# wei-zeng98/piano-a2s

Measured on AMD Instinct MI355X. Metric: training clips/sec (12 s, 5-bar), higher is better.
Workload: dtype f32

## Files before the change

### piano_a2s_amd/csrc/a2s_api.hip

```cpp
#define A2S_SWITCHES_IMPL
#include "a2s_internal.h"

thread_local char a2s_err_msg[512] = {0};
long long a2s_launch_counter = 0;

#define ST ((hipStream_t)stream)

extern "C" {

const char* a2s_last_error(void) { return a2s_err_msg; }
int a2s_version(void) { return 1; }
long long a2s_launch_count(void) { return __atomic_load_n(&a2s_launch_counter, __ATOMIC_RELAXED); }

int a2s_gemm_f32(void* stream, int M, int N, int K, float alpha, const float* A, long sAm, long sAk, const float* B, long sBk,
                 long sBn, float beta, float* C, long ldc, const float* bias, int act, int batch, long bsA, long bsB, long bsC,
                 int splitk, float* workspace, size_t workspace_bytes) {
    return a2s_gemm_impl(ST, M, N, K, alpha, A, sAm, sAk, B, sBk, sBn, beta, C, ldc, bias, act, batch, bsA, bsB, bsC, splitk,
                         workspace, workspace_bytes);
}
int a2s_gemm_f32_affine(void* stream, int M, int N, int K, float alpha, const float* A, long sAm, long sAk, const float* B, long sBk,
                        long sBn, float beta, float* C, long ldc, const float* bias, int act, int batch, long bsA, long bsB, long bsC,
                        int splitk, float* workspace, size_t workspace_bytes, const float* a_scale, const float* a_shift, int a_period,
                        const float* b_scale, const float* b_shift, int b_period) {
    return a2s_gemm_affine_impl(ST, M, N, K, alpha, A, sAm, sAk, B, sBk, sBn, beta, C, ldc, bias, act, batch, bsA, bsB, bsC, splitk,
// ... 32 lines not shown
}
size_t a2s_linear_wgrad_ws_bytes(int M, int K) { return a2s_linear_wgrad_ws_bytes_impl(M, K); }
int a2s_linear_wgrad_eligible(int M, int N, int K, int period) { return a2s_linear_wgrad_ok(M, N, K, 256, 4, 4, period, nullptr, nullptr, nullptr) ? 1 : 0; }
int a2s_tallk_wgrad(void* stream, int M, int Np, int K, const float* P, long ldp, const float* A, long lda, float* G, long ldg, int transposed, float* bias,
                    const float* p_absmax, const float* a_absmax, float* workspace, size_t workspace_bytes) {
    return a2s_tallk_wgrad_impl(ST, M, Np, K, P, ldp, A, lda, G, ldg, transposed, bias, p_absmax, a_absmax, workspace, workspace_bytes);
}
size_t a2s_tallk_wgrad_ws_bytes(int M, int Np, int K) { return a2s_tallk_wgrad_ws_bytes_impl(M, Np, K); }
int a2s_tallk_wgrad_eligible(int M, int Np, int K, long ldp, long lda, long ldg, int transposed) {
    return a2s_tallk_wgrad_ok(M, Np, K, ldp, lda, ldg, transposed, nullptr, nullptr, nullptr, nullptr) ? 1 : 0;
}
int a2s_linear_fwd_eligible(int M, int N, int K, int period) { return a2s_linear_fwd_ok(M, N, K, 4, 4, period, nullptr, nullptr, nullptr) ? 1 : 0; }
int a2s_linear_dgrad_blocks(int M) { return a2s_linear_dgrad_blocks_impl(M); }
int a2s_linear_dgrad_eligible(int M, int N, int K, int period) {
    return a2s_linear_dgrad_ok(M, N, K, 4, 1, K, 4, period, nullptr, nullptr, nullptr, nullptr) ? 1 : 0;
}
int a2s_gemm_f32_bnstats(void* stream, int M, int N, int K, const float* A, long sAm, long sAk, const float* B, long sBk, long sBn, float* C, long ldc,
                         const float* y, const float* mean, const float* invstd, const float* scale, const float* shift, int period, float* partial) {
    return a2s_gemm_affine_impl(ST, M, N, K, 1.f, A, sAm, sAk, B, sBk, sBn, 0.f, C, ldc, nullptr, 0, 1, 0, 0, 0, 1, nullptr, 0,
                                nullptr, nullptr, 0, nullptr, nullptr, 0, y, mean, invstd, scale, shift, partial, period, 0, nullptr, nullptr);
}
int a2s_gemm_bnstats_blocks(int M, int period) { return a2s_cdiv(M, 128) * a2s_gemm_bnstats_slots(period); }
size_t a2s_gemm_workspace_bytes(int M, int N, int batch, int splitk) { return a2s_gemm_workspace_bytes_impl(M, N, batch, splitk); }
int a2s_gemm_pick_splitk(int M, int N, int K, int batch) { return a2s_gemm_pick_splitk_impl(M, N, K, batch); }
void a2s_gemm_debug_tile(int cfg) { a2s_gemm_debug_tile_impl(cfg); }
size_t a2s_note_step_workspace_floats(int H, int E) { return a2s_note_step_workspace_floats_impl(H, E); }
int a2s_debug_set(const char* key, int value) {
    if (!key) return A2S_ERR_ARG;
    const int id = a2s_switch_find(key);
    if (id >= 0) { a2s_switch_store(id, value); return A2S_OK; }
    if (!strcmp(key, "attn_deferred_fast")) { a2s_attn_deferred_fast = value ? 1 : 0; return A2S_OK; }
    if (!strcmp(key, "tallk_wgrad")) { a2s_tallk_wgrad_on = value ? 1 : 0; return A2S_OK; }
    if (!strcmp(key, "tallk_wgrad_max_splits")) { a2s_tallk_wgrad_max_splits = value > 0 ? value : 0; return A2S_OK; }
    if (!strcmp(key, "gemm_tile")) { a2s_gemm_debug_tile_impl(value); return A2S_OK; }
    snprintf(a2s_err_msg, sizeof(a2s_err_msg), "a2s_debug_set: unknown key %s", key);
    return A2S_ERR_ARG;
}
int a2s_env_check(void) {
    if (const char* e = a2s_switch_env_error()) A2S_FAIL(A2S_ERR_ARG, "%s: expected a decimal number >= 0", e);
    return A2S_OK;
}

int a2s_persist_abort_latch(void* device_word) { a2s_persist_latch_set(device_word); return A2S_OK; }

int a2s_debug_get(const char* key) {
    if (!key) return -1;
    const int id = a2s_switch_find(key);
    if (id == A2S_SW_attn_pair_fused_rows) return a2s_attn_pair_fused_rows();
    if (id >= 0) return a2s_sw((a2s_switch)id);
    if (!strcmp(key, "attn_pair_launches")) return (int)a2s_attn_pair_launches();
    if (!strcmp(key, "attn_pair_bwd_launches")) return (int)a2s_attn_pair_bwd_launches();
    if (!strcmp(key, "attn_deferred_fast")) return a2s_attn_deferred_fast;
    if (!strcmp(key, "tallk_wgrad")) return a2s_tallk_wgrad_on;
    if (!strcmp(key, "tallk_wgrad_max_splits")) return a2s_tallk_wgrad_max_splits;
    if (!strcmp(key, "tallk_wgrad_launches")) return (int)a2s_tallk_wgrad_launches();
    if (!strcmp(key, "attn_dk_ahead_launches")) return (int)a2s_attn_dk_ahead_launches();
    if (!strcmp(key, "attn_denc_launches")) return (int)a2s_attn_denc_launches();
    if (!strcmp(key, "dec_mid_launches")) return a2s_dec_mid_launches();
    if (!strcmp(key, "dec_cmb_launches")) return a2s_dec_cmb_launches();
    if (!strcmp(key, "dec_persist_launches")) return a2s_dec_persist_launches();
    if (!strcmp(key, "gru_persist_fwd_launches")) return (int)a2s_gru_persist_fwd_launches();
    if (!strcmp(key, "gru_persist_bwd_launches")) return (int)a2s_gru_persist_bwd_launches();
    if (!strcmp(key, "gru_step_fwd_launches")) return (int)a2s_gru_step_fwd_launches();
    if (!strcmp(key, "gru_step_bwd_launches")) return (int)a2s_gru_step_bwd_launches();
    if (!strcmp(key, "edit_distance_launches")) return (int)a2s_edit_distance_launches();
    if (!strcmp(key, "conv_rows16_c20_launches")) return (int)a2s_conv_rows16_c20_launches();
    if (!strcmp(key, "device_cus")) return a2s_device_geometry().cus;
    if (!strcmp(key, "device_xccs")) return a2s_device_geometry().xccs;
    return -1;
}

int a2s_conv3x3(void* stream, const float* x, const float* w, float* y, const float* in_scale, const float* in_shift,
                float* stat_partial, int B, int T, int F, int Cin, int Cout, int flip, float* workspace) {
    return a2s_conv3x3_impl(ST, x, w, y, in_scale, in_shift, stat_partial, B, T, F, Cin, Cout, flip, workspace, nullptr, nullptr, nullptr, nullptr, nullptr, nullptr,
                            nullptr, nullptr);
}
int a2s_conv3x3_ranged(void* stream, const float* x, const float* w, float* y, const float* in_scale, const float* in_shift, const float* in_absmax,
                       float* stat_partial, float* out_absmax, int B, int T, int F, int Cin, int Cout, float* workspace) {
    return a2s_conv3x3_impl(ST, x, w, y, in_scale, in_shift, stat_partial, B, T, F, Cin, Cout, 0, workspace, nullptr, nullptr, nullptr, nullptr, nullptr, nullptr,
                            in_absmax, out_absmax);
}
int a2s_conv3x3_dgrad_bnstats(void* stream, const float* dy, const float* w, float* g, const float* yl, const float* yl_mean, const float* yl_invstd,
                              const float* yl_scale, const float* yl_shift, float* stat_partial, int B, int T, int F, int Cin, int Cout,
                              float* workspace) {
    if (!yl) { snprintf(a2s_err_msg, sizeof(a2s_err_msg), "conv3x3_dgrad_bnstats: yl is required"); return A2S_ERR_ARG; }
    return a2s_conv3x3_impl(ST, dy, w, g, nullptr, nullptr, stat_partial, B, T, F, Cin, Cout, 1, workspace, yl, yl_mean, yl_invstd, yl_scale, yl_shift, nullptr, nullptr, nullptr);
}
int a2s_conv3x3_dgrad_bnstats_scaled(void* stream, const float* dy, const float* w, float* g, const float* yl, const float* yl_mean, const float* yl_invstd,
                                     const float* yl_scale, const float* yl_shift, float* stat_partial, int B, int T, int F, int Cin, int Cout,
                                     float* workspace, const float* dy_absmax) {
    if (!yl) { snprintf(a2s_err_msg, sizeof(a2s_err_msg), "conv3x3_dgrad_bnstats_scaled: yl is required"); return A2S_ERR_ARG; }
    return a2s_conv3x3_impl(ST, dy, w, g, nullptr, nullptr, stat_partial, B, T, F, Cin, Cout, 1, workspace, yl, yl_mean, yl_invstd, yl_scale, yl_shift, dy_absmax, nullptr, nullptr);
}
int a2s_conv3x3_dgrad_bnstats_ranged(void* stream, const float* dy, const float* w, float* g, const float* yl, const float* yl_mean, const float* yl_invstd,
                                     const float* yl_scale, const float* yl_shift, float* stat_partial, int B, int T, int F, int Cin, int Cout,
                                     float* workspace, const float* dy_absmax, float* g_absmax_out) {
    if (!yl) { snprintf(a2s_err_msg, sizeof(a2s_err_msg), "conv3x3_dgrad_bnstats_ranged: yl is required"); return A2S_ERR_ARG; }
    return a2s_conv3x3_impl(ST, dy, w, g, nullptr, nullptr, stat_partial, B, T, F, Cin, Cout, 1, workspace, yl, yl_mean, yl_invstd, yl_scale, yl_shift, dy_absmax, nullptr, g_absmax_out);
}
// ... 395 lines not shown
```

### piano_a2s_amd/csrc/a2s_conv_rows.hip

```cpp
#include "a2s_internal.h"
#include <type_traits>

#define RW_P 120
#define RW_SROW 288
#define RW_SLOTS 5
#ifndef RW_EB
#define RW_EB 4
#endif
#define RW_HDR 160

typedef short s16x4 __attribute__((ext_vector_type(4)));
typedef short s16x8 __attribute__((ext_vector_type(8)));
#define RW_LDS(p) ((__attribute__((address_space(3))) s16x4*)(p))

template <int CIN>
struct RwGeom {
    static constexpr int NB = CIN / 4;
    static constexpr int KS = (3 * NB + 7) / 8;
    static constexpr int TS = CIN * RW_SROW;
    static constexpr int SLOT = 2 * TS + (CIN % 8 ? 128 : 0);
    static constexpr int ITEMS = CIN * 32;
    static constexpr int XIT = (ITEMS + 255) / 256;
};

// ... 518 lines not shown
        if (co >= 0)
            for (int e = tid; e < CIN * 9; e += 256) m = fmaxf(m, fabsf(weight(co, e / 9, e % 9)));
        m = block_max(m, red);
        if (tid == 0) {
            kw[c] = pow2_scale_exp(m, 13);
            if (co >= 0 && df == 0) hdr[80 + co] = ldexpf(1.f, -kw[c]);
        }
        __syncthreads();
    }
    for (int idx = tid; idx < G::KS * 512; idx += 256) {
        const int s = idx / 512, lane = (idx >> 3) & 63, e8 = idx & 7;
        const int li = lane & 15, g = lane >> 4, r = e8 >> 2, e = e8 & 3;
        const int kb = 8 * s + 4 * r + g;
        int co, df;
        column(li, co, df);
        float v = 0.f;
        if (co >= 0 && kb < 3 * G::NB) v = ldexpf(weight(co, 4 * (kb % G::NB) + e, (kb / G::NB) * 3 + df), kw[li]);
        unsigned t0, t1;
        split2_pair_f16(v, 0.f, t0, t1);
        unsigned short* dst = reinterpret_cast<unsigned short*>(wimg + ((size_t)(tile * G::KS + s) * 2) * 1024 + lane * 16 + e8 * 2);
        dst[0] = (unsigned short)t0;
        dst[512] = (unsigned short)t1;
    }
}

__device__ __forceinline__ float rw_ror8(float x) {
    return __int_as_float(__builtin_amdgcn_update_dpp(0, __float_as_int(x), 0x128, 0xf, 0xf, true));
}
__device__ __forceinline__ float rw_rol4(float x) {
    return __int_as_float(__builtin_amdgcn_update_dpp(0, __float_as_int(x), 0x12c, 0xf, 0xf, true));
}

#define R16_SLOTS 4
template <int CIN, int COUT, bool AFFINE, bool BNRED, bool PIPE = false>
__global__ __launch_bounds__(512, 2) void conv3x3_rows16(RowsArgs a) {
    using G = RwGeom<CIN>;
    using N = R16Geom<COUT>;
    constexpr int NTHR = 512, KS = G::KS;
    constexpr int WNM = N::WNM, NNT = N::NNT;
    constexpr bool B1L = PIPE || (CIN == 20 && COUT == 20 && BNRED);
    constexpr int XIT = (G::ITEMS + NTHR - 1) / NTHR;
    __shared__ __attribute__((aligned(16))) unsigned char ring[R16_SLOTS * G::SLOT];
    __shared__ __attribute__((aligned(16))) unsigned char b1img[B1L ? N::NTILES * G::KS * 1024 : 16];
    __shared__ float xch[2][N::NBND][2][16];
    __shared__ float red[8][16][3];
    __shared__ float tab[(AFFINE ? 2 * CIN : 0) + (BNRED ? 4 * COUT : 0) + 4];
    __shared__ __attribute__((aligned(16))) unsigned char dump[(G::ITEMS % NTHR) ? NTHR * 16 : 16];

    const int tid = threadIdx.x, lane = tid & 63;
    const int wave = __builtin_amdgcn_readfirstlane(tid >> 6);
    const int q = lane & 15, g = lane >> 4;
    const bool wide = wave < 4;
    const int wg = wave / N::WSPLIT, rng = wave % N::WSPLIT;
    const int m0 = wide ? WNM * rng : 2 * (wave - 4);
    const int nm = wide ? WNM : 2;
    const int tile0 = wide ? 3 * wg : 3 * N::NWG;
    const bool neg = wave & 1;
    const float sg = neg ? -1.f : 1.f;
    const int bnd_l = wide ? (rng > 0 ? wg * (N::WSPLIT - 1) + rng - 1 : -1) : (wave > 4 ? N::NWB + wave - 5 : -1);
    const int bnd_r = wide ? (rng < N::WSPLIT - 1 ? wg * (N::WSPLIT - 1) + rng : -1) : (wave < 7 ? N::NWB + wave - 4 : -1);

    int bid = blockIdx.x;
    {
        const int per = (int)gridDim.x / 8;
        if (bid < per * 8) bid = (bid % 8) * per + bid / 8;
    }
    const int ft = bid % a.tilesF; bid /= a.tilesF;
    const int strip = bid % a.nstrips, b = bid / a.nstrips;
    const int f_base = ft * RW_P;
    const int t_lo = strip * a.strip_len, t_hi = min(a.T, t_lo + a.strip_len);

    const unsigned sgn = neg ? 0x80008000u : 0u;
    constexpr int BWT = B1L ? 1 : 2;
    s16x8 bw[3][KS][BWT];
#pragma unroll
    for (int d = 0; d < 3; ++d)
#pragma unroll
        for (int s = 0; s < KS; ++s)
#pragma unroll
            for (int tm = 0; tm < BWT; ++tm) {
// ... 7 lines not shown
    }
    auto bterm1 = [&](int d, int s) -> s16x8 {
        if (B1L) {
            uint4 v = *reinterpret_cast<const uint4*>(b1img + ((tile0 + ((wide || d < NNT) ? d : 0)) * KS + s) * 1024 + lane * 16);
            v.x ^= sgn; v.y ^= sgn; v.z ^= sgn; v.w ^= sgn;
            return __builtin_bit_cast(s16x8, v);
        }
        return bw[d][s][BWT - 1];
    };
    const int co = wide ? wg * 16 + q : 16 * N::NWG + (q & (N::R - 1));
    const bool useful = wide || q < N::R;
    const float xscale = a.hdr[120];
    const float unsc = useful ? a.hdr[80 + co] / xscale * sg : 0.f;
    if (AFFINE && tid < 2 * CIN) tab[tid] = a.hdr[tid < CIN ? tid : 40 + tid - CIN];
    if (BNRED && tid < 4 * COUT) {
        const float* src = tid < COUT ? a.yl_mean : tid < 2 * COUT ? a.yl_invstd : tid < 3 * COUT ? a.yl_scale : a.yl_shift;
        tab[tid] = src[tid % COUT];
    }
    __syncthreads();
    float bm = 0.f, bi = 0.f, bsc = 0.f, bsh = 0.f;
    if (BNRED && useful) { bm = tab[co]; bi = tab[COUT + co]; bsc = tab[2 * COUT + co]; bsh = tab[3 * COUT + co]; }
    f32x2 st_s = {0.f, 0.f}, st_s2 = {0.f, 0.f};
    float st_m = 0.f;

    unsigned aaddr[KS][2];
#pragma unroll
    for (int s = 0; s < KS; ++s)
#pragma unroll
        for (int r = 0; r < 2; ++r) {
            int dt, cb;
            rw_block<CIN>(8 * s + 4 * r + g, dt, cb);
            aaddr[s][r] = (unsigned)(dt * G::SLOT + (4 * cb + q / 4) * RW_SROW + (q % 4) * 8 + m0 * 32);
        }
    const float* __restrict__ xclip = a.x + (long)b * a.T * CIN * a.F;
    const __amdgpu_buffer_rsrc_t xrsrc = __builtin_amdgcn_make_buffer_rsrc(const_cast<float*>(xclip), 0, (unsigned)((long)a.T * CIN * a.F * 4), 0x00020000);
    typedef unsigned u32x4 __attribute__((ext_vector_type(4)));
    const int fcol = f_base - 4 + 4 * (tid & 31);
    const bool colok = fcol >= 0 && fcol < a.F;
    auto issue = [&](int row, f32x4 (&xr)[XIT]) {
        const int rbase = row * CIN * a.F + f_base - 4;
        int tl = tid;
        asm volatile("" : "+v"(tl));
#pragma unroll
        for (int it = 0; it < XIT; ++it) {
            const int e = tl + NTHR * it;
            const int goff = (e >> 5) * a.F + 4 * (e & 31) + rbase;
            xr[it] = __builtin_bit_cast(f32x4, __builtin_amdgcn_raw_buffer_load_b128(xrsrc, (colok && e < G::ITEMS) ? goff * 4 : -4, 0, 0));
        }
    };
    auto commit_item = [&](int it, bool ok, unsigned char* base, const f32x4& x) {
        int tl = tid;
        asm volatile("" : "+v"(tl));
        const int e = tl + NTHR * it;
        const bool has = (it + 1) * NTHR <= G::ITEMS || e < G::ITEMS;
        const int ch = has ? e >> 5 : 0;
        unsigned char* const p0 = has ? base + ch * RW_SROW + (e & 31) * 8 : dump + tl * 16;
        unsigned char* const p1 = has ? p0 + G::TS : p0 + 8;
        f32x4 v = x;
        if (AFFINE) {
            const float sc = tab[ch], sh = tab[CIN + ch];
#pragma unroll
            for (int k = 0; k < 4; ++k) v[k] = ok ? fmaxf(fmaf(v[k], sc, sh), 0.f) : 0.f;
        } else {
#pragma unroll
            for (int k = 0; k < 4; ++k) v[k] = ok ? v[k] * xscale : 0.f;
        }
        uint2 t0, t1;
        split2_pair_f16(v[0], v[1], t0.x, t1.x);
        split2_pair_f16(v[2], v[3], t0.y, t1.y);
        *reinterpret_cast<uint2*>(p0) = t0;
        *reinterpret_cast<uint2*>(p1) = t1;
    };

    f32x4 acc[WNM][3];
    auto dterm1 = [](auto WIDEc, const f32x4 t0, const f32x4 t1, int r) -> float {
        if constexpr (decltype(WIDEc)::value) return t1[r];
        else if constexpr (N::R == 8) return rw_ror8(t0[r]);
        else return rw_rol4(t0[r]);
    };
    auto dterm2 = [](auto WIDEc, const f32x4 t0, const f32x4 t1, const f32x4 t2, int r) -> float {
        if constexpr (decltype(WIDEc)::value) return t2[r];
        else if constexpr (N::R == 8) return t1[r];
        else return rw_ror8(t0[r]);
    };
    auto multiply = [&](auto NMc, auto NTc, int crow, int cslot, const f32x4 (&xr)[XIT]) {
        constexpr int NM = decltype(NMc)::value, NT = decltype(NTc)::value;
        const bool cok = crow >= 0 && crow < a.T && colok;
        unsigned char* const cbase = ring + cslot * G::SLOT;
#pragma unroll
        for (int i = 0; i < NM; ++i)
#pragma unroll
            for (int d = 0; d < NT; ++d) acc[i][d] = (f32x4){0.f, 0.f, 0.f, 0.f};
#pragma unroll
        for (int s = 0; s < KS; ++s) {
            s16x8 b1[NT];
#pragma unroll
            for (int d = 0; d < NT; ++d) b1[d] = bterm1(d, s);
#pragma unroll
            for (int ig = 0; ig < NM / 2; ++ig) {
                s16x8 av[2][2];
#pragma unroll
                for (int tm = 0; tm < 2; ++tm)
#pragma unroll
                    for (int ii = 0; ii < 2; ++ii) {
                        const int off = tm * G::TS + (ig * 2 + ii) * 32;
                        const s16x4 lo = __builtin_amdgcn_ds_read_tr16_b64_v4i16(RW_LDS(ring + aaddr[s][0] + off));
                        const s16x4 hi = __builtin_amdgcn_ds_read_tr16_b64_v4i16(RW_LDS(ring + aaddr[s][1] + off));
                        av[tm][ii] = __builtin_shufflevector(lo, hi, 0, 1, 2, 3, 4, 5, 6, 7);
                    }
#define R16_PRODUCT(TA, BV)                                                                                                  \
    _Pragma("unroll") for (int d = 0; d < NT; ++d)                                                                           \
        _Pragma("unroll") for (int ii = 0; ii < 2; ++ii)                                                                     \
            acc[ig * 2 + ii][d] = __builtin_amdgcn_mfma_f32_16x16x32_f16(__builtin_bit_cast(f16x8, av[TA][ii]), __builtin_bit_cast(f16x8, BV), acc[ig * 2 + ii][d], 0, 0, 0);
                R16_PRODUCT(1, bw[d][s][0])
                R16_PRODUCT(0, b1[d])
                R16_PRODUCT(0, bw[d][s][0])
#undef R16_PRODUCT
            }
#pragma unroll
            for (int it = 0; it < XIT; ++it)
                if (it * KS / XIT == s) commit_item(it, cok, cbase, xr[it]);
        }
    };
    auto advance = [&]() {
#pragma unroll
        for (int s = 0; s < KS; ++s)
#pragma unroll
            for (int r = 0; r < 2; ++r) {
                const unsigned n = aaddr[s][r] + G::SLOT;
                aaddr[s][r] = min(n, n - R16_SLOTS * G::SLOT);
            }
    };

    const int up_addr = (((g + 3) & 3) * 16 + q) * 4;
    const int dn_addr = (((g + 1) & 3) * 16 + q) * 4;
    unsigned okbits = 0;
#pragma unroll
    for (int i = 0; i < WNM; ++i) {
        const int p = 16 * (m0 + i) + 4 * g;
        if (useful && i < nm && p >= 4 && p < 4 + RW_P && f_base - 4 + p < a.F) okbits |= 1u << i;
    }
    const __amdgpu_buffer_rsrc_t yrsrc = __builtin_amdgcn_make_buffer_rsrc(a.y + (long)b * a.T * COUT * a.F, 0, (unsigned)((long)a.T * COUT * a.F * 4), 0x00020000);
    const __amdgpu_buffer_rsrc_t ylrsrc = __builtin_amdgcn_make_buffer_rsrc(const_cast<float*>(BNRED ? a.yl + (long)b * a.T * COUT * a.F : a.x), 0,
                                                                            BNRED ? (unsigned)((long)a.T * COUT * a.F * 4) : 0u, 0x00020000);
    const int yvo = (co * a.F + f_base - 4 + 16 * m0 + 4 * g) * 4;
    f32x4 ylv[BNRED ? WNM : 1];
    auto yl_fetch = [&](int t) {
        if (!BNRED) return;
        const int yrow_off = t * COUT * a.F * 4;
#pragma unroll
        for (int i = 0; i < WNM; ++i)
            if (i < nm) ylv[BNRED ? i : 0] = __builtin_bit_cast(f32x4, __builtin_amdgcn_raw_buffer_load_b128(ylrsrc, yvo + 64 * i, yrow_off, 0));
    };
    auto epilogue = [&](auto WIDEc, int t, int par) {
// ... 19 lines not shown
            const float us = ok ? unsc : 0.f;
            f32x4 d1;
#pragma unroll
            for (int r = 0; r < 4; ++r) d1[r] = dterm1(WIDEc, acc[i][0], acc[i][1], r);
            f32x4 o;
            o[0] = ((X[i] + d1[0]) + dterm2(WIDEc, acc[i][0], acc[i][1], acc[i][2], 1)) * us;
            o[1] = ((acc[i][0][0] + d1[1]) + dterm2(WIDEc, acc[i][0], acc[i][1], acc[i][2], 2)) * us;
            o[2] = ((acc[i][0][1] + d1[2]) + dterm2(WIDEc, acc[i][0], acc[i][1], acc[i][2], 3)) * us;
            o[3] = ((acc[i][0][2] + d1[3]) + Y[i]) * us;
            if (ok) __builtin_amdgcn_raw_buffer_store_b128(__builtin_bit_cast(u32x4, o), yrsrc, yvo + 64 * i, yrow_off, 0);
            if (BNRED) {
                const f32x4 xv = ylv[BNRED ? i : 0];
                f32x4 gm, xh;
#pragma unroll
                for (int k = 0; k < 4; ++k) {
                    gm[k] = (fmaf(xv[k], bsc, bsh) > 0.f) ? o[k] : 0.f;
                    xh[k] = fmaf(xv[k], bi, -bm * bi);
                }
                st_s += (f32x2){gm[0], gm[1]}; st_s += (f32x2){gm[2], gm[3]};
                st_s2 += (f32x2){gm[0], gm[1]} * (f32x2){xh[0], xh[1]}; st_s2 += (f32x2){gm[2], gm[3]} * (f32x2){xh[2], xh[3]};
                if (a.out_absmax) st_m = fmaxf(fmaxf(st_m, fmaxf(fabsf(o[0]), fabsf(o[1]))), fmaxf(fabsf(o[2]), fabsf(o[3])));
            } else {
                st_s += (f32x2){o[0], o[1]}; st_s += (f32x2){o[2], o[3]};
                st_s2 += (f32x2){o[0], o[1]} * (f32x2){o[0], o[1]}; st_s2 += (f32x2){o[2], o[3]} * (f32x2){o[2], o[3]};
                st_m = fmaxf(fmaxf(st_m, fmaxf(fabsf(o[0]), fabsf(o[1]))), fmaxf(fabsf(o[2]), fabsf(o[3])));
            }
        }
    };

    f32x4 xa[XIT];
#pragma unroll
    for (int r = 0; r < 3; ++r) {
        issue(t_lo - 1 + r, xa);
#pragma unroll
        for (int it = 0; it < XIT; ++it) commit_item(it, t_lo - 1 + r >= 0 && t_lo - 1 + r < a.T && colok, ring + r * G::SLOT, xa[it]);
    }
    issue(t_lo + 2, xa);
    __syncthreads();

    if constexpr (PIPE) {
        f32x4 accp[2][WNM][3];
#pragma unroll
        for (int e = 0; e < 2; ++e)
#pragma unroll
            for (int i = 0; i < WNM; ++i)
#pragma unroll
                for (int d = 0; d < 3; ++d) accp[e][i][d] = (f32x4){0.f, 0.f, 0.f, 0.f};
        auto yl_tile = [&](int i, int t) -> f32x4 {
            return __builtin_bit_cast(f32x4, __builtin_amdgcn_raw_buffer_load_b128(ylrsrc, yvo + 64 * i, t * COUT * a.F * 4, 0));
        };
        auto epi_tile = [&](auto WIDEc, auto SETc, int i, int t, float xl, float xr_, unsigned ob, const f32x4& ylt) {
            constexpr bool WIDE = decltype(WIDEc)::value;
            constexpr int SET = decltype(SETc)::value, NM = WIDE ? WNM : 2;
            const int yrow_off = t * COUT * a.F * 4;
            const float up_src = (g == 3) ? (i > 0 ? accp[SET][i > 0 ? i - 1 : 0][0][3] : xl) : accp[SET][i][0][3];
            const int in = i < NM - 1 ? i + 1 : NM - 1;
            const float dn_src = (g == 0) ? (i < NM - 1 ? dterm2(WIDEc, accp[SET][in][0], accp[SET][in][1], accp[SET][in][2], 0) : xr_) : dterm2(WIDEc, accp[SET][i][0], accp[SET][i][1], accp[SET][i][2], 0);
            const float X = __int_as_float(__builtin_amdgcn_ds_bpermute(up_addr, __float_as_int(up_src)));
            const float Y = __int_as_float(__builtin_amdgcn_ds_bpermute(dn_addr, __float_as_int(dn_src)));
            const bool ok = ob >> i & 1;
            const float us = ok ? unsc : 0.f;
            f32x4 d1;
#pragma unroll
            for (int r = 0; r < 4; ++r) d1[r] = dterm1(WIDEc, accp[SET][i][0], accp[SET][i][1], r);
            f32x4 o;
            o[0] = ((X + d1[0]) + dterm2(WIDEc, accp[SET][i][0], accp[SET][i][1], accp[SET][i][2], 1)) * us;
            o[1] = ((accp[SET][i][0][0] + d1[1]) + dterm2(WIDEc, accp[SET][i][0], accp[SET][i][1], accp[SET][i][2], 2)) * us;
            o[2] = ((accp[SET][i][0][1] + d1[2]) + dterm2(WIDEc, accp[SET][i][0], accp[SET][i][1], accp[SET][i][2], 3)) * us;
// ... 32 lines not shown
                for (int d = 0; d < NT; ++d) accp[CUR][i][d] = (f32x4){0.f, 0.f, 0.f, 0.f};
#pragma unroll
            for (int s = 0; s < KS; ++s) {
                f32x4 ylt[(BNRED && NM > KS) ? NM / KS : 1];
                if (BNRED) {
#pragma unroll
                    for (int i = 0; i < NM; ++i)
                        if (i * KS / NM == s) ylt[(NM > KS) ? i - s * NM / KS : 0] = yl_tile(i, max(t_e, t_lo));
                }
                s16x8 b1[NT];
#pragma unroll
                for (int d = 0; d < NT; ++d) b1[d] = bterm1(d, s);
#pragma unroll
                for (int ig = 0; ig < NM / 2; ++ig) {
                    s16x8 av[2][2];
#pragma unroll
                    for (int tm = 0; tm < 2; ++tm)
#pragma unroll
                        for (int ii = 0; ii < 2; ++ii) {
                            const int off = tm * G::TS + (ig * 2 + ii) * 32;
                            const s16x4 lo = __builtin_amdgcn_ds_read_tr16_b64_v4i16(RW_LDS(ring + aaddr[s][0] + off));
                            const s16x4 hi = __builtin_amdgcn_ds_read_tr16_b64_v4i16(RW_LDS(ring + aaddr[s][1] + off));
                            av[tm][ii] = __builtin_shufflevector(lo, hi, 0, 1, 2, 3, 4, 5, 6, 7);
                        }
#define R16P_PRODUCT(TA, BV)                                                                                                 \
    _Pragma("unroll") for (int d = 0; d < NT; ++d)                                                                           \
        _Pragma("unroll") for (int ii = 0; ii < 2; ++ii)                                                                     \
            accp[CUR][ig * 2 + ii][d] = __builtin_amdgcn_mfma_f32_16x16x32_f16(__builtin_bit_cast(f16x8, av[TA][ii]), __builtin_bit_cast(f16x8, BV), accp[CUR][ig * 2 + ii][d], 0, 0, 0);
                    R16P_PRODUCT(1, bw[d][s][0])
                    R16P_PRODUCT(0, b1[d])
                    R16P_PRODUCT(0, bw[d][s][0])
#undef R16P_PRODUCT
                }
#pragma unroll
                for (int it = 0; it < XIT; ++it)
                    if (it * KS / XIT == s) commit_item(it, cok, cbase, xr[it]);
#pragma unroll
                for (int i = 0; i < NM; ++i)
                    if (i * KS / NM == s) epi_tile(WIDEc, std::integral_constant<int, 1 - CUR>{}, i, t_e, xl, xr_, ob, ylt[(BNRED && NM > KS) ? i - s * NM / KS : 0]);
            }
        };
        int slot_w = 3;
        auto row = [&](auto CURc, int t) {
            constexpr int CUR = decltype(CURc)::value;
            if (wide) multiply_p(std::true_type{}, CURc, t - 1, t + 2, slot_w, xa);
            else multiply_p(std::false_type{}, CURc, t - 1, t + 2, slot_w, xa);
            const float d2first = wide ? accp[CUR][0][2][0] : dterm2(std::false_type{}, accp[CUR][0][0], accp[CUR][0][1], accp[CUR][0][2], 0);
            if (bnd_r >= 0 && g == 3) xch[CUR][bnd_r >= 0 ? bnd_r : 0][0][q] = (wide ? accp[CUR][WNM - 1][0][3] : accp[CUR][1][0][3]) * sg;
            if (bnd_l >= 0 && g == 0) xch[CUR][bnd_l >= 0 ? bnd_l : 0][1][q] = d2first * sg;
            __syncthreads();
            issue(t + 3, xa);
            slot_w = slot_w == R16_SLOTS - 1 ? 0 : slot_w + 1;
            advance();
        };
        using C0 = std::integral_constant<int, 0>; using C1 = std::integral_constant<int, 1>;
        int t = t_lo, last = 0;
        for (;;) {
            row(C0{}, t);
            if (++t >= t_hi) { last = 0; break; }
            row(C1{}, t);
            if (++t >= t_hi) { last = 1; break; }
        }
        {
            const float xl = bnd_l >= 0 ? xch[last][bnd_l >= 0 ? bnd_l : 0][0][q] * sg : 0.f;
            const float xr_ = bnd_r >= 0 ? xch[last][bnd_r >= 0 ? bnd_r : 0][1][q] * sg : 0.f;
            unsigned ob = okbits;
            asm volatile("" : "+v"(ob));
#pragma unroll
            for (int i = 0; i < WNM; ++i) {
                if (i < nm) {
                    const f32x4 ylt = BNRED ? yl_tile(i, t_hi - 1) : (f32x4){0.f, 0.f, 0.f, 0.f};
                    if (wide) { if (last) epi_tile(std::true_type{}, C1{}, i, t_hi - 1, xl, xr_, ob, ylt); else epi_tile(std::true_type{}, C0{}, i, t_hi - 1, xl, xr_, ob, ylt); }
                    else if (i < 2) { if (last) epi_tile(std::false_type{}, C1{}, i < 2 ? i : 0, t_hi - 1, xl, xr_, ob, ylt); else epi_tile(std::false_type{}, C0{}, i < 2 ? i : 0, t_hi - 1, xl, xr_, ob, ylt); }
                }
            }
        }
    } else {
    int slot_w = 3, par = 0;
#ifdef RW_TRACE
    const int rp = wave & 1, ng = wave >> 1;
    const int trace_first = (int)gridDim.x / 2;
    const int trace_wg = ((int)blockIdx.x >= trace_first && (int)blockIdx.x < trace_first + RW_TRACE_WGS) ? (int)blockIdx.x - trace_first : -1;
#endif
    using I2 = std::integral_constant<int, 2>; using I3 = std::integral_constant<int, 3>;
    using IW = std::integral_constant<int, WNM>; using INt = std::integral_constant<int, NNT>;
    for (int t = t_lo; t < t_hi; ++t) {
#ifdef RW_TRACE
        const int trace_it = t - t_lo - 40;
#endif
        RW_STAMP(0);
        yl_fetch(t);
        if (wide) multiply(IW{}, I3{}, t + 2, slot_w, xa);
        else multiply(I2{}, INt{}, t + 2, slot_w, xa);
        RW_STAMP(1);
        const float d2first = wide ? acc[0][2][0] : dterm2(std::false_type{}, acc[0][0], acc[0][1], acc[0][2], 0);
        if (bnd_r >= 0 && g == 3) xch[par][bnd_r >= 0 ? bnd_r : 0][0][q] = (wide ? acc[WNM - 1][0][3] : acc[1][0][3]) * sg;
        if (bnd_l >= 0 && g == 0) xch[par][bnd_l >= 0 ? bnd_l : 0][1][q] = d2first * sg;
        __syncthreads();
        RW_STAMP(2);
        if (wide) epilogue(std::true_type{}, t, par);
        else epilogue(std::false_type{}, t, par);
        RW_STAMP(3);
        issue(t + 3, xa);
        RW_STAMP(4);
        slot_w = slot_w == R16_SLOTS - 1 ? 0 : slot_w + 1;
        par ^= 1;
        advance();
    }
    }

    {
        float s = st_s[0] + st_s[1], s2 = st_s2[0] + st_s2[1], m = st_m;
        s += __shfl_xor(s, 16, 64); s2 += __shfl_xor(s2, 16, 64); m = fmaxf(m, __shfl_xor(m, 16, 64));
        s += __shfl_xor(s, 32, 64); s2 += __shfl_xor(s2, 32, 64); m = fmaxf(m, __shfl_xor(m, 32, 64));
        if (g == 0) { red[wave][q][0] = s; red[wave][q][1] = s2; red[wave][q][2] = m; }
    }
    __syncthreads();
    if (tid < COUT) {
        float s = 0.f, s2 = 0.f, m = 0.f;
        constexpr int CW = 16 * N::NWG;
        const int w0 = tid < CW ? N::WSPLIT * (tid >> 4) : 4, nw = tid < CW ? N::WSPLIT : 4, c = tid < CW ? tid & 15 : tid - CW;
        for (int k = 0; k < nw; ++k) { s += red[w0 + k][c][0]; s2 += red[w0 + k][c][1]; m = fmaxf(m, red[w0 + k][c][2]); }
        if (a.stat_partial) {
            a.stat_partial[((long)blockIdx.x * COUT + tid) * 2 + 0] = s;
            a.stat_partial[((long)blockIdx.x * COUT + tid) * 2 + 1] = s2;
        }
        if (a.out_absmax) {
            const unsigned bits = __float_as_uint(m);
            if (bits > __hip_atomic_load(reinterpret_cast<unsigned*>(a.out_absmax + tid), __ATOMIC_RELAXED, __HIP_MEMORY_SCOPE_AGENT))
                atomicMax(reinterpret_cast<unsigned*>(a.out_absmax + tid), bits);
        }
    }
}

bool a2s_conv_rows_eligible(int F, int Cin) { return a2s_sw(A2S_SW_conv_rows) && F % 4 == 0 && (Cin == 20 || Cin == 40); }

static void rows_geometry(int B, int T, int F, int* tilesF, int* nstrips, int* strip_len) {
    *tilesF = a2s_cdiv(F, RW_P);
    int ns = a2s_cdiv(2048, (long)B * *tilesF);
    ns = ns < 1 ? 1 : ns;
    const int max_ns = T / 16 > 1 ? T / 16 : 1;
    ns = ns > max_ns ? max_ns : ns;
    int len = a2s_cdiv(T, ns);
    len += len & 1;
    *strip_len = len;
    *nstrips = a2s_cdiv(T, len);
}
int a2s_conv_rows_blocks(int B, int T, int F) {
    int tf, ns, len;
    rows_geometry(B, T, F, &tf, &ns, &len);
    return B * tf * ns;
}
size_t a2s_conv_rows_workspace_floats(int Cin) {
    return (size_t)9 * RwGeom<40>::KS * 2 * 1024 / 4 + RW_HDR + 64;
}

static long long g_rows16_c20_launches = 0;
long a2s_conv_rows16_c20_launches(void) { return (long)__atomic_load_n(&g_rows16_c20_launches, __ATOMIC_RELAXED); }

template <int CIN, int COUT>
static int rows16_launch(hipStream_t st, const RowsArgs& a, bool affine, bool bnred, int nwork) {
    constexpr int NT = 512;
    if (COUT == 20) __atomic_fetch_add(&g_rows16_c20_launches, 1LL, __ATOMIC_RELAXED);
    constexpr bool SETS2 = !(CIN == 20 && COUT == 20);
    const int en = SETS2 ? a2s_sw(A2S_SW_conv_rows) : 0;
    if (affine && (en & 4)) hipLaunchKernelGGL((conv3x3_rows16<CIN, COUT, true, false, SETS2>), dim3(nwork), dim3(NT), 0, st, a);
    else if (affine) hipLaunchKernelGGL((conv3x3_rows16<CIN, COUT, true, false>), dim3(nwork), dim3(NT), 0, st, a);
    else if (bnred && (en & 8)) hipLaunchKernelGGL((conv3x3_rows16<CIN, COUT, false, true, SETS2>), dim3(nwork), dim3(NT), 0, st, a);
    else if (bnred) hipLaunchKernelGGL((conv3x3_rows16<CIN, COUT, false, true>), dim3(nwork), dim3(NT), 0, st, a);
    else hipLaunchKernelGGL((conv3x3_rows16<CIN, COUT, false, false>), dim3(nwork), dim3(NT), 0, st, a);
    A2S_CHECK_LAUNCH("conv3x3_rows16");
    return A2S_OK;
}
template <int CIN, int COUT>
static int rows_launch(hipStream_t st, const RowsArgs& a, bool affine, bool bnred, int nwork) {
    if (affine) hipLaunchKernelGGL((conv3x3_rows<CIN, COUT, true, false>), dim3(nwork), dim3(512), 0, st, a);
    else if (bnred) hipLaunchKernelGGL((conv3x3_rows<CIN, COUT, false, true>), dim3(nwork), dim3(512), 0, st, a);
    else hipLaunchKernelGGL((conv3x3_rows<CIN, COUT, false, false>), dim3(nwork), dim3(512), 0, st, a);
    A2S_CHECK_LAUNCH("conv3x3_rows");
    return A2S_OK;
}
template <int CIN, int COUT>
static void rows_pack_launch(hipStream_t st, const float* w, int flip, const float* in_scale, const float* in_shift, const float* in_absmax,
                             const float* x_absmax, unsigned char* wimg, float* hdr, float* out_absmax) {
    hipLaunchKernelGGL((rows_pack<CIN, COUT>), dim3(COUT / 5), dim3(256), 0, st, w, flip, in_scale, in_shift, in_absmax, x_absmax, wimg, hdr, out_absmax);
}

int a2s_conv3x3_rows_impl(hipStream_t st, const float* x, const float* w, float* y, const float* in_scale, const float* in_shift,
                          const float* in_absmax, float* stat_partial, float* out_absmax, int B, int T, int F, int Cin, int Cout, int flip,
                          float* ws, const float* yl, const float* yl_mean, const float* yl_invstd, const float* yl_scale, const float* yl_shift,
                          const float* x_absmax) {
    A2S_REQUIRE(F % 4 == 0 && (Cin == 20 || Cin == 40) && (Cout == 20 || Cout == 40), "conv3x3_rows: unsupported shape F=%d Cin=%d Cout=%d", F, Cin, Cout);
    A2S_REQUIRE(!(in_scale && yl), "conv3x3_rows: input affine and BatchNorm-backward statistics are exclusive");
    const bool gen2 = a2s_sw(A2S_SW_conv_rows) & 2;
    if (yl && Cin == 20 && Cout == 20 && out_absmax && !gen2) {
        const int rc = a2s_conv3x3_rows_impl(st, x, w, y, in_scale, in_shift, in_absmax, stat_partial, nullptr, B, T, F, Cin, Cout, flip, ws, yl, yl_mean, yl_invstd,
                                             yl_scale, yl_shift, x_absmax);
        return rc != A2S_OK ? rc : a2s_channel_absmax_impl(st, y, (long)B * T, Cout, F, out_absmax);
    }
    unsigned char* wimg = reinterpret_cast<unsigned char*>(ws);
    float* hdr = ws + (size_t)9 * RwGeom<40>::KS * 2 * 1024 / 4;
    float* scratch = hdr + RW_HDR;
    if (in_scale && !in_absmax) {
// ... 32 lines not shown
```

### piano_a2s_amd/csrc/a2s_internal.h

```cpp
#pragma once
#include "a2s_common.h"
#include "../../include/a2s.h"
#include "a2s_switches.h"

static inline int a2s_attn_pair_fused_rows(void) {
    const int cap = a2s_sw(A2S_SW_dec_fused_max_rows), v = a2s_sw(A2S_SW_attn_pair_fused_rows);
    return v < cap ? v : cap;
}
static inline unsigned a2s_persist_dbg(void) {
    return (a2s_sw(A2S_SW_persist_force_agent) ? PERSIST_DBG_FORCE_AGENT : 0u) | (a2s_sw(A2S_SW_persist_inject_abort) ? PERSIST_DBG_INJECT_ABORT : 0u);
}

int a2s_absmax_impl(hipStream_t st, const float* x, long n, float* out);
size_t a2s_gemm_workspace_bytes_impl(int M, int N, int batch, int splitk);
int a2s_gemm_pick_splitk_impl(int M, int N, int K, int batch);
int a2s_gemm_bnstats_slots(int period);
void a2s_gemm_debug_tile_impl(int cfg);
int a2s_gemm_affine_impl(hipStream_t st, int M, int N, int K, float alpha, const float* A, long sAm, long sAk,
    const float* B, long sBk, long sBn, float beta, float* C, long ldc, const float* bias, int act,
    int batch, long bsA, long bsB, long bsC, int splitk, float* ws, size_t ws_bytes,
    const float* a_scale, const float* a_shift, int a_period, const float* b_scale, const float* b_shift, int b_period,
    const float* ep_y, const float* ep_mean, const float* ep_invstd, const float* ep_scale, const float* ep_shift,
    float* ep_partial, int ep_period, int two_term, const float* a_absmax, const float* b_absmax);
int a2s_gemm_impl(hipStream_t st, int M, int N, int K, float alpha, const float* A, long sAm, long sAk,
// ... 31 lines not shown
int a2s_bn_finalize_impl(hipStream_t st, const float* partial, int nblocks, int C, double count, const float* gamma,
    const float* beta, float* running_mean, float* running_var, long long* nbt, float* mean,
    float* invstd, float* scale, float* shift, float eps, float momentum, int training);
int a2s_bn_relu_apply_impl(hipStream_t st, const float* x, float* y, const float* scale, const float* shift, long n, int C, int F);
int a2s_col_stats_impl(hipStream_t st, const float* x, float* partial, long rows, int C, int rows_per_block);
int a2s_bn1d_relu_dropout_impl(hipStream_t st, const float* x, float* y, const float* scale, const float* shift,
    const uint8_t* mask, float inv_keep, long n, int C);
size_t a2s_conv3x3_wgrad_workspace_bytes_impl(int Cin, int Cout);
int a2s_conv3x3_wgrad_impl(hipStream_t st, const float* dy, const float* x, const float* in_scale, const float* in_shift, float* dW,
    float* ws, size_t ws_bytes, int B, int T, int F, int Cin, int Cout, const float* bn_y, const float* bn_mean,
    const float* bn_invstd, const float* bn_scale, const float* bn_shift, const float* bn_c12, float* dy_out,
    const float* dy_absmax, const float* act_absmax);
int a2s_bn_bwd_impl(hipStream_t st, const float* g, const float* x, const float* mean, const float* invstd, const float* scale,
    const float* shift, const uint8_t* mask, float inv_keep, float* dgamma, float* dbeta, float* dx, float* partial,
    float* c12, long rows, int C, int F, float* dx_absmax);
int a2s_bn_bwd_from_partial_impl(hipStream_t st, const float* g, const float* x, const float* mean, const float* invstd, const float* scale,
    const float* shift, float* dgamma, float* dbeta, float* dx, const float* partial, int nblocks, float* c12,
    long rows, int C, int F, float* dx_absmax);
int a2s_bn_bwd_stats_impl(hipStream_t st, const float* g, const float* x, const float* mean, const float* invstd, const float* scale,
    const float* shift, const uint8_t* mask, float inv_keep, float* partial, float* sums, long rows, int C, int F);
int a2s_bn_bwd_apply_impl(hipStream_t st, const float* g, const float* x, const float* mean, const float* invstd, const float* scale,
    const float* shift, const uint8_t* mask, float inv_keep, const float* sums_local, const float* sums_global,
    double count_global, float* dgamma, float* dbeta, float* dx, float* c12, long rows, int C, int F);
int a2s_bn_bwd_sums_from_partial_impl(hipStream_t st, const float* partial, int nblocks, int C, float* sums);
int a2s_bn_bwd_c12_from_sums_impl(hipStream_t st, const float* sums_local, const float* sums_global, double count_global, float* dgamma, float* dbeta,
    float* c12, int C);
size_t a2s_bn_bwd_partial_floats_impl(long rows, int C, int F);

int a2s_channel_absmax_impl(hipStream_t st, const float* x, long rows, int C, int F, float* out);
bool a2s_conv_rows_eligible(int F, int Cin);
int a2s_conv_rows_blocks(int B, int T, int F);
size_t a2s_conv_rows_workspace_floats(int Cin);
long a2s_conv_rows16_c20_launches(void);
int a2s_conv3x3_rows_impl(hipStream_t st, const float* x, const float* w, float* y, const float* in_scale, const float* in_shift,
    const float* in_absmax, float* stat_partial, float* out_absmax, int B, int T, int F, int Cin, int Cout, int flip,
    float* ws, const float* yl, const float* yl_mean, const float* yl_invstd, const float* yl_scale, const float* yl_shift,
    const float* x_absmax);

bool a2s_wgrad_rows_eligible(int F, int Cin, int Cout);
int a2s_conv3x3_wgrad_rows_bn_impl(hipStream_t st, const float* g, const float* y, const float* mean, const float* invstd, const float* scale,
    const float* shift, const float* c12, const float* g_absmax, int g_absmax_n, const float* y_absmax, float* dz_out,
    float* dz_absmax_out, const float* x, const float* in_scale, const float* in_shift, float* dW, float* ws, size_t ws_bytes,
    int B, int T, int F, int Cin, int Cout, const float* act_absmax);
int a2s_conv3x3_wgrad_rows_impl(hipStream_t st, const float* dy, const float* x, const float* in_scale, const float* in_shift, float* dW, float* ws,
    size_t ws_bytes, int B, int T, int F, int Cin, int Cout, const float* dy_absmax, const float* act_absmax);

struct StepFinArgs {
    const float* logits; long ldl;
    float* probs; long probs_bstride;
    const long long* gt; long gt_bstride;
    const float* emb;
    float* xnext; long ldx;
    const uint8_t* drop; float inv_keep;
    int* argmax_out; long am_bstride;
    int* eos_seen; long long* lengths; int* n_done; int* steps_exec;
    const int* t_base;
    const int* row_until;
    int n_clips;
    int R, V, E, t, teacher_force, eos_id, max_t;
};
struct a2s_grammar_ref { const signed char* next; int n_states; int* row_state; };
struct a2s_metre_ref { const int* dur_ticks; const uint8_t* cls; const uint8_t* fillable; int n_fillable; int* row_metre; };
int a2s_gru_gates_fwd_impl(hipStream_t st, const float* gi, long ldgi, const float* gh, long ldgh, const float* hprev,
    long ldhp, float* hout, long ldho, float* hout2, long ldho2, float* save, int R, int H);
int a2s_gru_bptt_step_impl(hipStream_t st, const float* dgh, const float* w_hh_t, const float* dhz_in, const float* dout, long ld_dout,
    const float* save, const float* hprev, long ld_hprev, float* dgi, long ld_dgi, float* dgh_out, float* dgh2,
// ... 277 lines not shown
```

Before: 634.1.

## Stage conv rows input loads only on narrow waves in rows16 kernel

```diff
diff --git a/piano_a2s_amd/csrc/a2s_api.hip b/piano_a2s_amd/csrc/a2s_api.hip
--- a/piano_a2s_amd/csrc/a2s_api.hip
+++ b/piano_a2s_amd/csrc/a2s_api.hip
@@ -88,6 +88,7 @@
     if (!strcmp(key, "attn_deferred_fast")) { a2s_attn_deferred_fast = value ? 1 : 0; return A2S_OK; }
     if (!strcmp(key, "tallk_wgrad")) { a2s_tallk_wgrad_on = value ? 1 : 0; return A2S_OK; }
     if (!strcmp(key, "tallk_wgrad_max_splits")) { a2s_tallk_wgrad_max_splits = value > 0 ? value : 0; return A2S_OK; }
+    if (!strcmp(key, "conv_rows_stage")) { a2s_conv_rows_stage = value & 3; return A2S_OK; }
     if (!strcmp(key, "gemm_tile")) { a2s_gemm_debug_tile_impl(value); return A2S_OK; }
     snprintf(a2s_err_msg, sizeof(a2s_err_msg), "a2s_debug_set: unknown key %s", key);
     return A2S_ERR_ARG;
@@ -121,6 +122,8 @@
     if (!strcmp(key, "gru_step_bwd_launches")) return (int)a2s_gru_step_bwd_launches();
     if (!strcmp(key, "edit_distance_launches")) return (int)a2s_edit_distance_launches();
     if (!strcmp(key, "conv_rows16_c20_launches")) return (int)a2s_conv_rows16_c20_launches();
+    if (!strcmp(key, "conv_rows_stage")) return a2s_conv_rows_stage;
+    if (!strcmp(key, "conv_rows_stage_launches")) return (int)a2s_conv_rows_stage_launches();
     if (!strcmp(key, "device_cus")) return a2s_device_geometry().cus;
     if (!strcmp(key, "device_xccs")) return a2s_device_geometry().xccs;
     return -1;
diff --git a/piano_a2s_amd/csrc/a2s_conv_rows.hip b/piano_a2s_amd/csrc/a2s_conv_rows.hip
--- a/piano_a2s_amd/csrc/a2s_conv_rows.hip
+++ b/piano_a2s_amd/csrc/a2s_conv_rows.hip
@@ -574,20 +574,21 @@
 }
 
 #define R16_SLOTS 4
-template <int CIN, int COUT, bool AFFINE, bool BNRED, bool PIPE = false>
+template <int CIN, int COUT, bool AFFINE, bool BNRED, bool PIPE = false, bool SN = false>
 __global__ __launch_bounds__(512, 2) void conv3x3_rows16(RowsArgs a) {
     using G = RwGeom<CIN>;
     using N = R16Geom<COUT>;
     constexpr int NTHR = 512, KS = G::KS;
     constexpr int WNM = N::WNM, NNT = N::NNT;
     constexpr bool B1L = PIPE || (CIN == 20 && COUT == 20 && BNRED);
-    constexpr int XIT = (G::ITEMS + NTHR - 1) / NTHR;
+    constexpr int NSTG = SN ? 256 : NTHR;
+    constexpr int XIT = (G::ITEMS + NSTG - 1) / NSTG;
     __shared__ __attribute__((aligned(16))) unsigned char ring[R16_SLOTS * G::SLOT];
     __shared__ __attribute__((aligned(16))) unsigned char b1img[B1L ? N::NTILES * G::KS * 1024 : 16];
     __shared__ float xch[2][N::NBND][2][16];
     __shared__ float red[8][16][3];
     __shared__ float tab[(AFFINE ? 2 * CIN : 0) + (BNRED ? 4 * COUT : 0) + 4];
-    __shared__ __attribute__((aligned(16))) unsigned char dump[(G::ITEMS % NTHR) ? NTHR * 16 : 16];
+    __shared__ __attribute__((aligned(16))) unsigned char dump[(G::ITEMS % NSTG) ? NSTG * 16 : 16];
 
     const int tid = threadIdx.x, lane = tid & 63;
     const int wave = __builtin_amdgcn_readfirstlane(tid >> 6);
@@ -661,27 +662,30 @@
             rw_block<CIN>(8 * s + 4 * r + g, dt, cb);
             aaddr[s][r] = (unsigned)(dt * G::SLOT + (4 * cb + q / 4) * RW_SROW + (q % 4) * 8 + m0 * 32);
         }
+    const bool stager = !SN || !wide;
+    const int stid = SN ? tid - (NTHR - NSTG) : tid;
     const float* __restrict__ xclip = a.x + (long)b * a.T * CIN * a.F;
     const __amdgpu_buffer_rsrc_t xrsrc = __builtin_amdgcn_make_buffer_rsrc(const_cast<float*>(xclip), 0, (unsigned)((long)a.T * CIN * a.F * 4), 0x00020000);
     typedef unsigned u32x4 __attribute__((ext_vector_type(4)));
     const int fcol = f_base - 4 + 4 * (tid & 31);
     const bool colok = fcol >= 0 && fcol < a.F;
     auto issue = [&](int row, f32x4 (&xr)[XIT]) {
+        if (!stager) return;
         const int rbase = row * CIN * a.F + f_base - 4;
-        int tl = tid;
+        int tl = stid;
         asm volatile("" : "+v"(tl));
 #pragma unroll
         for (int it = 0; it < XIT; ++it) {
-            const int e = tl + NTHR * it;
+            const int e = tl + NSTG * it;
             const int goff = (e >> 5) * a.F + 4 * (e & 31) + rbase;
             xr[it] = __builtin_bit_cast(f32x4, __builtin_amdgcn_raw_buffer_load_b128(xrsrc, (colok && e < G::ITEMS) ? goff * 4 : -4, 0, 0));
         }
     };
     auto commit_item = [&](int it, bool ok, unsigned char* base, const f32x4& x) {
-        int tl = tid;
+        int tl = stid;
         asm volatile("" : "+v"(tl));
-        const int e = tl + NTHR * it;
-        const bool has = (it + 1) * NTHR <= G::ITEMS || e < G::ITEMS;
+        const int e = tl + NSTG * it;
+        const bool has = (it + 1) * NSTG <= G::ITEMS || e < G::ITEMS;
         const int ch = has ? e >> 5 : 0;
         unsigned char* const p0 = has ? base + ch * RW_SROW + (e & 31) * 8 : dump + tl * 16;
         unsigned char* const p1 = has ? p0 + G::TS : p0 + 8;
@@ -746,9 +750,11 @@
                 R16_PRODUCT(0, bw[d][s][0])
 #undef R16_PRODUCT
             }
-#pragma unroll
-            for (int it = 0; it < XIT; ++it)
-                if (it * KS / XIT == s) commit_item(it, cok, cbase, xr[it]);
+            if constexpr (!SN || NT == NNT) {
+#pragma unroll
+                for (int it = 0; it < XIT; ++it)
+                    if (it * KS / XIT == s) commit_item(it, cok, cbase, xr[it]);
+            }
         }
     };
     auto advance = [&]() {
@@ -834,8 +840,10 @@
 #pragma unroll
     for (int r = 0; r < 3; ++r) {
         issue(t_lo - 1 + r, xa);
-#pragma unroll
-        for (int it = 0; it < XIT; ++it) commit_item(it, t_lo - 1 + r >= 0 && t_lo - 1 + r < a.T && colok, ring + r * G::SLOT, xa[it]);
+        if (stager) {
+#pragma unroll
+            for (int it = 0; it < XIT; ++it) commit_item(it, t_lo - 1 + r >= 0 && t_lo - 1 + r < a.T && colok, ring + r * G::SLOT, xa[it]);
+        }
     }
     issue(t_lo + 2, xa);
     __syncthreads();
@@ -934,24 +942,30 @@
                     R16P_PRODUCT(0, bw[d][s][0])
 #undef R16P_PRODUCT
                 }
-#pragma unroll
-                for (int it = 0; it < XIT; ++it)
-                    if (it * KS / XIT == s) commit_item(it, cok, cbase, xr[it]);
+                if constexpr (!SN || !WIDE) {
+#pragma unroll
+                    for (int it = 0; it < XIT; ++it)
+                        if (it * KS / XIT == s) commit_item(it, cok, cbase, xr[it]);
+                }
 #pragma unroll
                 for (int i = 0; i < NM; ++i)
                     if (i * KS / NM == s) epi_tile(WIDEc, std::integral_constant<int, 1 - CUR>{}, i, t_e, xl, xr_, ob, ylt[(BNRED && NM > KS) ? i - s * NM / KS : 0]);
             }
         };
+        auto rows_p = [&](auto ROLEc) {
+        constexpr int ROLE = decltype(ROLEc)::value;
+        const bool w = ROLE == 0 ? wide : ROLE == 1;
+        const int nmr = ROLE == 0 ? nm : ROLE == 1 ? WNM : 2;
         int slot_w = 3;
         auto row = [&](auto CURc, int t) {
             constexpr int CUR = decltype(CURc)::value;
-            if (wide) multiply_p(std::true_type{}, CURc, t - 1, t + 2, slot_w, xa);
+            if (w) multiply_p(std::true_type{}, CURc, t - 1, t + 2, slot_w, xa);
             else multiply_p(std::false_type{}, CURc, t - 1, t + 2, slot_w, xa);
-            const float d2first = wide ? accp[CUR][0][2][0] : dterm2(std::false_type{}, accp[CUR][0][0], accp[CUR][0][1], accp[CUR][0][2], 0);
-            if (bnd_r >= 0 && g == 3) xch[CUR][bnd_r >= 0 ? bnd_r : 0][0][q] = (wide ? accp[CUR][WNM - 1][0][3] : accp[CUR][1][0][3]) * sg;
+            const float d2first = w ? accp[CUR][0][2][0] : dterm2(std::false_type{}, accp[CUR][0][0], accp[CUR][0][1], accp[CUR][0][2], 0);
+            if (bnd_r >= 0 && g == 3) xch[CUR][bnd_r >= 0 ? bnd_r : 0][0][q] = (w ? accp[CUR][WNM - 1][0][3] : accp[CUR][1][0][3]) * sg;
             if (bnd_l >= 0 && g == 0) xch[CUR][bnd_l >= 0 ? bnd_l : 0][1][q] = d2first * sg;
             __syncthreads();
-            issue(t + 3, xa);
+            if (ROLE != 1) issue(t + 3, xa);
             slot_w = slot_w == R16_SLOTS - 1 ? 0 : slot_w + 1;
             advance();
         };
@@ -970,15 +984,19 @@
             asm volatile("" : "+v"(ob));
 #pragma unroll
             for (int i = 0; i < WNM; ++i) {
-                if (i < nm) {
+                if (i < nmr) {
                     const f32x4 ylt = BNRED ? yl_tile(i, t_hi - 1) : (f32x4){0.f, 0.f, 0.f, 0.f};
-                    if (wide) { if (last) epi_tile(std::true_type{}, C1{}, i, t_hi - 1, xl, xr_, ob, ylt); else epi_tile(std::true_type{}, C0{}, i, t_hi - 1, xl, xr_, ob, ylt); }
+                    if (w) { if (last) epi_tile(std::true_type{}, C1{}, i, t_hi - 1, xl, xr_, ob, ylt); else epi_tile(std::true_type{}, C0{}, i, t_hi - 1, xl, xr_, ob, ylt); }
                     else if (i < 2) { if (last) epi_tile(std::false_type{}, C1{}, i < 2 ? i : 0, t_hi - 1, xl, xr_, ob, ylt); else epi_tile(std::false_type{}, C0{}, i < 2 ? i : 0, t_hi - 1, xl, xr_, ob, ylt); }
                 }
             }
         }
+        };
+        if constexpr (SN) {
+            if (wide) rows_p(std::integral_constant<int, 1>{});
+            else rows_p(std::integral_constant<int, 2>{});
+        } else rows_p(std::integral_constant<int, 0>{});
     } else {
-    int slot_w = 3, par = 0;
 #ifdef RW_TRACE
     const int rp = wave & 1, ng = wave >> 1;
     const int trace_first = (int)gridDim.x / 2;
@@ -986,29 +1004,38 @@
 #endif
     using I2 = std::integral_constant<int, 2>; using I3 = std::integral_constant<int, 3>;
     using IW = std::integral_constant<int, WNM>; using INt = std::integral_constant<int, NNT>;
+    auto rows = [&](auto ROLEc) {
+    constexpr int ROLE = decltype(ROLEc)::value;
+    const bool w = ROLE == 0 ? wide : ROLE == 1;
+    int slot_w = 3, par = 0;
     for (int t = t_lo; t < t_hi; ++t) {
 #ifdef RW_TRACE
         const int trace_it = t - t_lo - 40;
 #endif
         RW_STAMP(0);
         yl_fetch(t);
-        if (wide) multiply(IW{}, I3{}, t + 2, slot_w, xa);
+        if (w) multiply(IW{}, I3{}, t + 2, slot_w, xa);
         else multiply(I2{}, INt{}, t + 2, slot_w, xa);
         RW_STAMP(1);
-        const float d2first = wide ? acc[0][2][0] : dterm2(std::false_type{}, acc[0][0], acc[0][1], acc[0][2], 0);
-        if (bnd_r >= 0 && g == 3) xch[par][bnd_r >= 0 ? bnd_r : 0][0][q] = (wide ? acc[WNM - 1][0][3] : acc[1][0][3]) * sg;
+        const float d2first = w ? acc[0][2][0] : dterm2(std::false_type{}, acc[0][0], acc[0][1], acc[0][2], 0);
+        if (bnd_r >= 0 && g == 3) xch[par][bnd_r >= 0 ? bnd_r : 0][0][q] = (w ? acc[WNM - 1][0][3] : acc[1][0][3]) * sg;
         if (bnd_l >= 0 && g == 0) xch[par][bnd_l >= 0 ? bnd_l : 0][1][q] = d2first * sg;
         __syncthreads();
         RW_STAMP(2);
-        if (wide) epilogue(std::true_type{}, t, par);
+        if (w) epilogue(std::true_type{}, t, par);
         else epilogue(std::false_type{}, t, par);
         RW_STAMP(3);
-        issue(t + 3, xa);
+        if (ROLE != 1) issue(t + 3, xa);
         RW_STAMP(4);
         slot_w = slot_w == R16_SLOTS - 1 ? 0 : slot_w + 1;
         par ^= 1;
         advance();
     }
+    };
+    if constexpr (SN) {
+        if (wide) rows(std::integral_constant<int, 1>{});
+        else rows(std::integral_constant<int, 2>{});
+    } else rows(std::integral_constant<int, 0>{});
     }
 
     {
@@ -1060,17 +1087,38 @@
 static long long g_rows16_c20_launches = 0;
 long a2s_conv_rows16_c20_launches(void) { return (long)__atomic_load_n(&g_rows16_c20_launches, __ATOMIC_RELAXED); }
 
+int a2s_conv_rows_stage = 3;
+static long long g_rows_stage_launches = 0;
+long a2s_conv_rows_stage_launches(void) { return (long)__atomic_load_n(&g_rows_stage_launches, __ATOMIC_RELAXED); }
+constexpr bool rows16_stage_narrow(int cin, int cout, bool affine, bool bnred, bool pipe) {
+#ifdef R16_SN_ALL
+    return true;
+#else
+    return !(bnred && ((cin == 20 && cout == 20) || (cin == 20 && cout == 40) || (cin == 40 && cout == 20 && pipe)));
+#endif
+}
+
+template <int CIN, int COUT, bool AFFINE, bool BNRED, bool PIPE>
+static void rows16_launch_form(hipStream_t st, const RowsArgs& a, int nwork) {
+    if constexpr (rows16_stage_narrow(CIN, COUT, AFFINE, BNRED, PIPE)) {
+        if (a2s_conv_rows_stage & 1) {
+            __atomic_fetch_add(&g_rows_stage_launches, 1LL, __ATOMIC_RELAXED);
+            hipLaunchKernelGGL((conv3x3_rows16<CIN, COUT, AFFINE, BNRED, PIPE, true>), dim3(nwork), dim3(512), 0, st, a);
+            return;
+        }
+    }
+    hipLaunchKernelGGL((conv3x3_rows16<CIN, COUT, AFFINE, BNRED, PIPE, false>), dim3(nwork), dim3(512), 0, st, a);
+}
 template <int CIN, int COUT>
 static int rows16_launch(hipStream_t st, const RowsArgs& a, bool affine, bool bnred, int nwork) {
-    constexpr int NT = 512;
     if (COUT == 20) __atomic_fetch_add(&g_rows16_c20_launches, 1LL, __ATOMIC_RELAXED);
     constexpr bool SETS2 = !(CIN == 20 && COUT == 20);
     const int en = SETS2 ? a2s_sw(A2S_SW_conv_rows) : 0;
-    if (affine && (en & 4)) hipLaunchKernelGGL((conv3x3_rows16<CIN, COUT, true, false, SETS2>), dim3(nwork), dim3(NT), 0, st, a);
-    else if (affine) hipLaunchKernelGGL((conv3x3_rows16<CIN, COUT, true, false>), dim3(nwork), dim3(NT), 0, st, a);
-    else if (bnred && (en & 8)) hipLaunchKernelGGL((conv3x3_rows16<CIN, COUT, false, true, SETS2>), dim3(nwork), dim3(NT), 0, st, a);
-    else if (bnred) hipLaunchKernelGGL((conv3x3_rows16<CIN, COUT, false, true>), dim3(nwork), dim3(NT), 0, st, a);
-    else hipLaunchKernelGGL((conv3x3_rows16<CIN, COUT, false, false>), dim3(nwork), dim3(NT), 0, st, a);
+    if (affine && (en & 4)) rows16_launch_form<CIN, COUT, true, false, SETS2>(st, a, nwork);
+    else if (affine) rows16_launch_form<CIN, COUT, true, false, false>(st, a, nwork);
+    else if (bnred && ((en & 8) || (CIN == 40 && COUT == 40 && (a2s_conv_rows_stage & 3) == 3))) rows16_launch_form<CIN, COUT, false, true, SETS2>(st, a, nwork);
+    else if (bnred) rows16_launch_form<CIN, COUT, false, true, false>(st, a, nwork);
+    else rows16_launch_form<CIN, COUT, false, false, false>(st, a, nwork);
     A2S_CHECK_LAUNCH("conv3x3_rows16");
     return A2S_OK;
 }
diff --git a/piano_a2s_amd/csrc/a2s_internal.h b/piano_a2s_amd/csrc/a2s_internal.h
--- a/piano_a2s_amd/csrc/a2s_internal.h
+++ b/piano_a2s_amd/csrc/a2s_internal.h
@@ -87,6 +87,8 @@
 int a2s_conv_rows_blocks(int B, int T, int F);
 size_t a2s_conv_rows_workspace_floats(int Cin);
 long a2s_conv_rows16_c20_launches(void);
+extern int a2s_conv_rows_stage;
+long a2s_conv_rows_stage_launches(void);
 int a2s_conv3x3_rows_impl(hipStream_t st, const float* x, const float* w, float* y, const float* in_scale, const float* in_shift,
     const float* in_absmax, float* stat_partial, float* out_absmax, int B, int T, int F, int Cin, int Cout, int flip,
     float* ws, const float* yl, const float* yl_mean, const float* yl_invstd, const float* yl_scale, const float* yl_shift,
```

Result: faster. 646.5 (median of 6 runs) (+2.0%).
